# Klaudiusz321/raytracing-engine-in-c

Measured on AMD Instinct MI355X. Metric: Mrays/s (and RK4 steps/s) per GPU + per node; max |Δhit| vs CPU ref, higher is better.
Workload: dtype f64

## Files before the change

include/bhrt_api.h:

```cpp
#ifndef BHRT_API_H
#define BHRT_API_H

#include "bhrt_types.h"

#ifdef __cplusplus
extern "C" {
#endif

#define BLACKHOLE_API_VERSION_MAJOR 0
#define BLACKHOLE_API_VERSION_MINOR 1
#define BLACKHOLE_API_VERSION_PATCH 0

#define BH_PI 3.14159265358979323846
#define BH_EPSILON 1.0e-10
#define BH_TWO_PI 6.28318530717958647692

typedef enum {
    BH_SUCCESS = 0,
    BH_ERROR_INVALID_PARAMETER = -1,
    BH_ERROR_MEMORY_ALLOCATION = -2,
    BH_ERROR_INITIALIZATION = -3,
    BH_ERROR_SIMULATION = -4
} BHErrorCode;

// ... 263 lines not shown
    int64_t frames_total;
    int64_t pixels;
} bhrt_accum_state;

typedef struct {
    uint8_t* rgba8;
    float*   rgb;
    float*   edge_factor;
} bhrt_accum_out;

float bhrt_accum_alpha(const bhrt_accum_params* params, int frame_count);

int bhrt_accum_create(int width, int height, const bhrt_rows* rows, const bhrt_accum_params* params,
                      bhrt_accum** acc);

void bhrt_accum_destroy(bhrt_accum* acc);

int bhrt_accum_reset(bhrt_accum* acc);

int bhrt_accum_info(const bhrt_accum* acc, const SupersamplingParams* ss, bhrt_accum_state* state);

int bhrt_accum_device_buffers(const bhrt_accum* acc, const float** device_rgb,
                              const float** device_edge);

int bhrt_accum_frame_device(bhrt_accum* acc, const BlackHoleParams* blackhole,
                            const AccretionDiskParams* disk, const SimulationConfig* config,
                            const bhrt_camera* camera, IntegrationMethod method, int flags,
                            const SupersamplingParams* ss, const bhrt_accum_out* device_out,
                            void* hip_stream);

int bhrt_accum_blend_device(bhrt_accum* acc, const float* device_rgb,
                            const bhrt_accum_out* device_out, void* hip_stream);

int bhrt_accum_frame(bhrt_accum* acc, const BlackHoleParams* blackhole,
                     const AccretionDiskParams* disk, const SimulationConfig* config,
                     const bhrt_camera* camera, IntegrationMethod method, int flags,
                     const SupersamplingParams* ss, const bhrt_accum_out* host_out);

int bhrt_render_frame_async(const BlackHoleParams* blackhole, const AccretionDiskParams* disk,
                            const SimulationConfig* config, const bhrt_camera* camera, int width,
                            int height, IntegrationMethod method, int flags,
                            const bhrt_frame_soa* host_out, int* ticket);

int bhrt_frame_wait(int ticket);

int bhrt_trace_rays_device(const Ray* device_rays, int n, const BlackHoleParams* blackhole,
                           const AccretionDiskParams* disk, const SimulationConfig* config,
                           IntegrationMethod method, int flags,
                           const bhrt_frame_soa* device_out, void* hip_stream);

int bhrt_trace_rays(const Ray* rays, int n, const BlackHoleParams* blackhole,
                    const AccretionDiskParams* disk, const SimulationConfig* config,
                    IntegrationMethod method, int flags, const bhrt_frame_soa* host_out);

#define BHRT_PATHS_MAX_POSITIONS 65536

typedef struct {
    Vector3D* xyz;
    float*    xyz32;
    int32_t*  count;
} bhrt_paths;

int bhrt_trace_paths_device(const Ray* device_rays, int n, const BlackHoleParams* blackhole,
                            const AccretionDiskParams* disk, const SimulationConfig* config,
                            IntegrationMethod method, int max_positions, int every,
                            const bhrt_paths* device_paths, const bhrt_frame_soa* device_hits,
                            void* hip_stream);

int bhrt_trace_paths(const Ray* rays, int n, const BlackHoleParams* blackhole,
                     const AccretionDiskParams* disk, const SimulationConfig* config,
                     IntegrationMethod method, int max_positions, int every,
                     const bhrt_paths* host_paths, const bhrt_frame_soa* host_hits);

int bhrt_check_rkf45_accept(const double* err, const double* scale, const double* tol, int n,
                            int* out, void* hip_stream);

int bhrt_check_disk_hit(const double* p, const double* d, const double* nrm, int n, double in_sq,
                        double out_sq, int* out, void* hip_stream);

int bhrt_check_seg_len(const double* x, int n, double* out, void* hip_stream);

int bhrt_check_pair_rcp(const double* in, int n, int huge, double* out, void* hip_stream);

int bhrt_get_stats(bhrt_stats* out, int reset);

int bhrt_device_count(void);

void bhrt_set_refill_threshold(int lanes);

int bhrt_set_claim_order(const int* d_order, int n);

int bhrt_update_particles_steps(ParticleSystem* system, const BlackHoleParams* blackhole,
                                const SimulationConfig* config, int steps, double* kernel_ms);

const char* bhrt_last_error(void);

#ifdef __cplusplus
}
#endif
#endif
```

raytracing-engine-in-c_amd/csrc/geodesic.hip:

```cpp
#include <hip/hip_runtime.h>

#include <atomic>
#include <type_traits>

#include "bhrt_kernel.h"

#pragma clang fp contract(fast)

namespace {

constexpr double kEps = 1.0e-10;
constexpr double kTwoPi = 6.28318530717958647692;

using Scene = bhrt_scene_k;

constexpr int kStopMark = (int)0x80000000u;
struct Counters {
    unsigned rays = 0, iters = 0, full = 0, far_ = 0, kerr = 0;
    bool huge = false;
    int mark = 0;
    __device__ __forceinline__ void raise_huge() {
        huge = true;
        mark = kStopMark;
    }
// ... 63 lines not shown
    constexpr double S1 = -1.66666666666666324348e-01, S2 = 8.33333333332248946124e-03,
                     S3 = -1.98412698298579493134e-04, S4 = 2.75573137070700676789e-06,
                     S5 = -2.50507602534068634195e-08, S6 = 1.58969099521155010221e-10;
    constexpr double C1 = 4.16666666666666019037e-02, C2 = -1.38888888888741095749e-03,
                     C3 = 2.48015872894767294178e-05, C4 = -2.75573143513906633035e-07,
                     C5 = 2.08757232129817482790e-09, C6 = -1.13596475577881948265e-11;
    const double z = r * r, w = z * z;
    const double rs_ = fmac_k(z, fmac_k(z, S4, S3), S2) + z * w * fmac_k(z, S6, S5);
    const double v = z * r;
    const double s = r - ((z * (0.5 * y - v * rs_) - y) - v * S1);
    const double rc = z * fmac_k(z, fmac_k(z, C3, C2), C1) +
                      w * w * fmac_k(z, fmac_k(z, C6, C5), C4);
    const double hz = 0.5 * z, ww = 1.0 - hz;
    const double c = ww + (((1.0 - ww) - hz) + (z * rc - r * y));
    const int q = (int)n;
    double ss = (q & 1) ? c : s;
    double cc = (q & 1) ? s : c;
    *so = (q & 2) ? -ss : ss;
    *co = ((q + 1) & 2) ? -cc : cc;
}

__device__ __forceinline__ bool sincos_shift_wide(double a, double s0, double c0, double x,
                                                  double& s, double& c) {
    const double delta = x - a;
    if (!(fabs(delta) <= 0.78539816339744828 && fabs(delta) <= 0.5 * fabs(a))) return false;
    constexpr double S1 = -1.66666666666666324348e-01, S2 = 8.33333333332248946124e-03,
                     S3 = -1.98412698298579493134e-04, S4 = 2.75573137070700676789e-06,
                     S5 = -2.50507602534068634195e-08, S6 = 1.58969099521155010221e-10;
    constexpr double C1 = 4.16666666666666019037e-02, C2 = -1.38888888888741095749e-03,
                     C3 = 2.48015872894767294178e-05, C4 = -2.75573143513906633035e-07,
                     C5 = 2.08757232129817482790e-09, C6 = -1.13596475577881948265e-11;
    const double z = delta * delta, w = z * z;
    const double r = fmac_k(z, fmac_k(z, S4, S3), S2) + z * w * fmac_k(z, S6, S5);
    const double sd = delta + (z * delta) * fmac_k(z, r, S1);
    const double rc = z * fmac_k(z, fmac_k(z, C3, C2), C1) +
                      w * w * fmac_k(z, fmac_k(z, C6, C5), C4);
    const double cm1 = z * rc - 0.5 * z;
    s = s0 + (s0 * cm1 + c0 * sd);
    c = c0 + (c0 * cm1 - s0 * sd);
    return true;
}

__device__ __forceinline__ void rotation_coeffs(double delta, double& sd, double& cm1) {
    const double z = delta * delta;
    if (__builtin_expect(fabs(delta) <= 0.0625, 1)) {
        constexpr double S1 = -0.16666666666662605, S2 = 0.00833333327878775,
                         S3 = -0.00019839069723619096;
        constexpr double C1 = 0.04166666666666157, C2 = -0.0013888888827212717,
                         C3 = 2.479927034006378e-05;
        sd = delta + (z * delta) * fmac_k(z, fmac_k(z, S3, S2), S1);
        cm1 = z * __builtin_fma(z, fmac_k(z, fmac_k(z, C3, C2), C1), -0.5);
        return;
    }
    constexpr double S1 = -1.66666666666666324348e-01, S2 = 8.33333333332248946124e-03,
                     S3 = -1.98412698298579493134e-04, S4 = 2.75573137070700676789e-06,
                     S5 = -2.50507602534068634195e-08, S6 = 1.58969099521155010221e-10;
    constexpr double C1 = 4.16666666666666019037e-02, C2 = -1.38888888888741095749e-03,
                     C3 = 2.48015872894767294178e-05, C4 = -2.75573143513906633035e-07,
                     C5 = 2.08757232129817482790e-09, C6 = -1.13596475577881948265e-11;
    const double w = z * z;
    const double r = fmac_k(z, fmac_k(z, S4, S3), S2) + z * w * fmac_k(z, S6, S5);
    sd = delta + (z * delta) * fmac_k(z, r, S1);
    const double rc = z * fmac_k(z, fmac_k(z, C3, C2), C1) + w * w * fmac_k(z, fmac_k(z, C6, C5), C4);
    cm1 = z * rc - 0.5 * z;
}

__device__ __forceinline__ void shift_or_eval(double a, double s0, double c0, double x, double& s,
                                              double& c, Counters* hc) {
    const double delta = x - a;
    constexpr double S1 = -0.16666666666662605, S2 = 0.00833333327878775,
                     S3 = -0.00019839069723619096;
    constexpr double C1 = 0.04166666666666157, C2 = -0.0013888888827212717,
                     C3 = 2.479927034006378e-05;
    const double z = delta * delta;
    const double sd = delta + (z * delta) * fmac_k(z, fmac_k(z, S3, S2), S1);
    const double cm1 = z * __builtin_fma(z, fmac_k(z, fmac_k(z, C3, C2), C1), -0.5);
    s = __builtin_fma(c0, sd, __builtin_fma(s0, cm1, s0));
    c = __builtin_fma(-s0, sd, __builtin_fma(c0, cm1, c0));
    if (__builtin_expect(!(fabs(delta) <= 0.0625), 0)) {
        if (!sincos_shift_wide(a, s0, c0, x, s, c)) bhrt_sincos(x, &s, &c, hc);
    }
}

struct Trig1 {
    double a, s, c;
};

__device__ __forceinline__ void accel_literal(const double (&y)[6], double (&d)[6], const Scene& sc,
                                              double st, double ct) {
    double r = y[0];
    double rsq = r * r;
    double st2 = st * st;
    if (r <= sc.rs_x1_5) {
        r = sc.rs_x1_5;
        rsq = r * r;
    }
    if (fabs(st) < 0.01) {
        st = (st >= 0.0) ? 0.01 : -0.01;
        st2 = st * st;
    }
    const double term2 = r * y[4] * y[4];
    const double term3 = r * st2 * y[5] * y[5];
    const double n4 = -2.0 * y[3] * y[4];
    const double n5a = -2.0 * y[3] * y[5];
    const double n5b = 2.0 * y[4] * y[5] * ct;
    const double sc4 = st * ct * y[5] * y[5];
    if (r < 1.0e150) {
        const double yr = rcp_nr(r);
        const double term1 = -(sc.M * yr) * yr;
        d[3] = term1 + term2 + term3;
        d[4] = div_nr(n4, r, yr) + sc4;
        d[5] = div_nr(n5a, r, yr) - div_nr(n5b, st, rcp_nr(st));
    } else {
        const double f = 1.0 - sc.rs / r;
        const double term1 = -sc.M / (rsq * f) * f;
        d[3] = term1 + term2 + term3;
        d[4] = n4 / r + sc4;
        d[5] = n5a / r - n5b / st;
    }
}

template <bool BOUNDED = false>
__device__ __forceinline__ void repair_clamp(double (&d)[6]) {
#pragma unroll
    for (int i = BOUNDED ? 3 : 0; i < 6; i++)
        if (!isfinite(d[i])) d[i] = 0.0;
#pragma unroll
    for (int i = 3; i < 6; i++) d[i] = fmin(fmax(d[i], -10.0), 10.0);
}

template <bool HUGE>
__device__ __forceinline__ void accel_fast(const double (&y)[6], double (&d)[6], const Scene& sc,
                                           double st, double ct, double rc, double w2, bool ok) {
    const double yr2 = st * w2, ys2 = rc * w2;
    const double u = st * y[5];
    const double f3 = rc * __builtin_fma(u, u, y[4] * y[4]);
    d[3] = __builtin_fma(-(sc.m_4 * yr2), yr2, f3);
    const double p2 = y[3] * yr2;
    d[4] = __builtin_fma(p2, y[4], u * (ct * y[5]));
    d[5] = y[5] * __builtin_fma(y[4], ct * ys2, p2);
    const int plain = (int)ok & (int)(fabs(d[3]) <= 10.0) & (int)(fabs(d[4]) <= 10.0) &
                      (int)(fabs(d[5]) <= 10.0);
    if (__builtin_expect(plain, 1)) return;
    accel_literal(y, d, sc, st, ct);
    repair_clamp<!HUGE>(d);
}

#ifndef BHRT_COUNT_STAGES
#define BHRT_COUNT_STAGES 0
#endif
template <bool SPIN0, bool FAR, bool HUGE>
__device__ __forceinline__ void rhs(const double (&y)[6], double (&d)[6], const Scene& sc,
                                    bool far_ok, Counters& n, Trig1& tr, bool first) {
    d[0] = y[3];
    d[1] = y[4];
    d[2] = y[5];
    if (FAR && far_ok && y[0] > sc.rs_x15) {
        d[3] = 0.0;
        d[4] = 0.0;
        d[5] = y[5] * (sc.two_m / (y[0] * y[0]));
        n.far_++;
        return;
    }
    if (SPIN0) {
        double st, ct;
        if (first) {
            st = tr.s;
            ct = tr.c;
        } else {
            shift_or_eval(tr.a, tr.s, tr.c, y[1], st, ct, HUGE ? nullptr : &n);
        }
        if ((FAR && HUGE) || BHRT_COUNT_STAGES) n.full++;
        const double rc = max_raw(y[0], sc.rs_x1_5);
        const bool ok = (!HUGE ? true : rc < 1.0e150) & (fabs(st) >= 0.01);
        accel_fast<HUGE>(y, d, sc, st, ct, rc, rcp_nr_m2(rc * st), ok);
        return;
    }
    d[3] = 0.0;
    d[4] = 0.0;
    d[5] = 0.0;
    if ((FAR && HUGE) || BHRT_COUNT_STAGES) n.kerr++;
    const int plain = (int)(fabs(d[3]) <= 10.0) & (int)(fabs(d[4]) <= 10.0) &
                      (int)(fabs(d[5]) <= 10.0);
    if (plain) return;
    repair_clamp<!HUGE>(d);
}

template <int METHOD, bool FAR, bool HUGE>
constexpr bool repair_at_refill() {
    return (METHOD == INTEGRATOR_RK4 || METHOD == INTEGRATOR_RKF45) && !HUGE;
}

template <bool SPIN0, bool FAR>
constexpr bool zero_accel() {
    return !SPIN0 && !FAR;
}

template <int METHOD, bool SPIN0, bool FAR, bool HUGE>
constexpr bool hoist_sums() {
    return METHOD == INTEGRATOR_RKF45 && zero_accel<SPIN0, FAR>() &&
           repair_at_refill<METHOD, FAR, HUGE>();
}

template <int METHOD, bool SPIN0, bool FAR, bool HUGE>
constexpr bool rotation_trig() {
    return zero_accel<SPIN0, FAR>() && repair_at_refill<METHOD, FAR, HUGE>() &&
           (METHOD == INTEGRATOR_RK4 || METHOD == INTEGRATOR_RKF45);
}

__device__ __forceinline__ double rk4_acc(double acc, double k) { return acc + 2.0 * k; }
constexpr double kC1 = 25.0 / 216.0, kC3 = 1408.0 / 2565.0, kC4 = 2197.0 / 4104.0,
                 kC5 = -1.0 / 5.0;
constexpr double kD1 = 16.0 / 135.0, kD3 = 6656.0 / 12825.0, kD4 = 28561.0 / 56430.0,
                 kD5 = -9.0 / 50.0, kD6 = 2.0 / 55.0;
__device__ __forceinline__ double rkf45_sum4(double k1, double k3, double k4, double k5) {
    return kC1 * k1 + kC3 * k3 + kC4 * k4 + kC5 * k5;
}
__device__ __forceinline__ double rkf45_sum5(double k1, double k3, double k4, double k5,
                                             double k6) {
    return kD1 * k1 + kD3 * k3 + kD4 * k4 + kD5 * k5 + kD6 * k6;
}

#ifndef BHRT_PAIR_RCP
#define BHRT_PAIR_RCP 1
#endif
struct StageOps {
    double st, ct, rc, x;
    bool ok;
};
template <bool HUGE>
__device__ __forceinline__ void stage_x(StageOps& o) {
    o.x = o.rc * o.st;
    o.ok = (!HUGE ? true : o.rc < 1.0e150) & (fabs(o.st) >= 0.01);
}
template <bool FAR, bool HUGE>
__device__ __forceinline__ void stage_ops(double y0, double y1, bool far, const Scene& sc,
                                          Counters& n, const Trig1& tr, StageOps& o) {
    shift_or_eval(tr.a, tr.s, tr.c, y1, o.st, o.ct, HUGE ? nullptr : &n);
    o.rc = max_raw(y0, sc.rs_x1_5);
    stage_x<HUGE>(o);
    if (FAR && far) {
        o.x = 1.0;
        o.ok = true;
    }
}
__device__ __forceinline__ bool pair_rcp(const StageOps& a, const StageOps& b, double& wa,
                                         double& wb) {
    const double w = rcp_nr_m2(a.x * b.x);
    wa = b.x * w;
    wb = a.x * w;
    return a.ok & b.ok;
}
template <bool FAR, bool HUGE>
__device__ __forceinline__ void rhs_given(const double (&y)[6], double (&d)[6], const Scene& sc,
                                          bool far, Counters& n, const StageOps& o, double w2,
                                          bool ok) {
    d[0] = y[3];
    d[1] = y[4];
    d[2] = y[5];
    if (FAR && far) {
        d[3] = 0.0;
        d[4] = 0.0;
        d[5] = y[5] * (sc.two_m / (y[0] * y[0]));
        n.far_++;
        return;
    }
    if ((FAR && HUGE) || BHRT_COUNT_STAGES) n.full++;
    accel_fast<HUGE>(y, d, sc, o.st, o.ct, o.rc, w2, ok);
}

template <bool SPIN0, bool FAR, bool HUGE, bool HS = false>
__device__ __forceinline__ void rk4_step(double (&y)[6], double h, double h6, const Scene& sc,
                                         bool far_ok, Counters& n, Trig1& tr,
                                         const double* zs = nullptr) {
    constexpr bool Z = zero_accel<SPIN0, FAR>();
    double k[6], acc[6], yt[6];
    const double hh = 0.5 * h;
    rhs<SPIN0, FAR, HUGE>(y, k, sc, far_ok, n, tr, true);
#pragma unroll
    for (int i = 0; i < 6; i++) {
        acc[i] = k[i];
        yt[i] = (Z && i >= 3) ? y[i] : y[i] + hh * k[i];
    }
    if constexpr (SPIN0 && BHRT_PAIR_RCP) {
        const double y30 = y[0] + hh * yt[3], y31 = y[1] + hh * yt[4];
        const bool far2 = FAR && far_ok && yt[0] > sc.rs_x15;
        const bool far3 = FAR && far_ok && y30 > sc.rs_x15;
        StageOps o2, o3;
        double w2 = 0.0, w3 = 0.0;
        bool ok = false;
        if (!FAR || !(far2 & far3)) {
            stage_ops<FAR, HUGE>(yt[0], yt[1], far2, sc, n, tr, o2);
            stage_ops<FAR, HUGE>(y30, y31, far3, sc, n, tr, o3);
            ok = pair_rcp(o2, o3, w2, w3);
        }
        rhs_given<FAR, HUGE>(yt, k, sc, far2, n, o2, w2, ok);
#pragma unroll
        for (int i = 0; i < 6; i++) {
            acc[i] = rk4_acc(acc[i], k[i]);
            yt[i] = i == 0 ? y30 : i == 1 ? y31 : y[i] + hh * k[i];
        }
        rhs_given<FAR, HUGE>(yt, k, sc, far3, n, o3, w3, ok);
    } else {
        rhs<SPIN0, FAR, HUGE>(yt, k, sc, far_ok, n, tr, false);
#pragma unroll
        for (int i = 0; i < 6; i++) {
            acc[i] = rk4_acc(acc[i], k[i]);
            yt[i] = (Z && i >= 3) ? y[i] : y[i] + hh * k[i];
        }
        rhs<SPIN0, FAR, HUGE>(yt, k, sc, far_ok, n, tr, false);
    }
#pragma unroll
    for (int i = 0; i < 6; i++) {
        acc[i] = rk4_acc(acc[i], k[i]);
        yt[i] = (Z && i >= 3) ? y[i] : y[i] + h * k[i];
    }
    rhs<SPIN0, FAR, HUGE>(yt, k, sc, far_ok, n, tr, false);
#pragma unroll
    for (int i = 0; i < 6; i++) {
        if (HS && i < 3)
            y[i] = __builtin_fma(h6, zs[i], y[i]);
        else if (!(Z && i >= 3))
            y[i] = __builtin_fma(h6, acc[i] + k[i], y[i]);
    }
}

template <bool FAST, int NC = 6>
__device__ __forceinline__ bool rkf45_accept(const double (&err)[6], const double (&scale)[6],
                                             double tol) {
    const bool tol_normal = tol >= 2.2250738585072014e-308 && tol <= 1.79769313486231570815e+308;
    if (FAST && tol >= 0x1p-900 && tol <= 0x1p300) {
        const double lo = tol * (1.0 - 0x1p-40), hi = tol * (1.0 + 0x1p-40);
        bool all_pass = true;
#pragma unroll
        for (int i = 0; i < NC; i++) all_pass &= err[i] <= lo * scale[i];
        if (__builtin_expect(all_pass, 1)) return true;
        double near_max = 0.0;
        bool over = false;
#pragma unroll
        for (int i = 0; i < NC; i++) {
            const bool pass = err[i] <= lo * scale[i];
            const bool fail = err[i] > hi * scale[i];
            over |= fail;
            if (__builtin_expect(!pass && !fail, 0)) near_max = fmax(near_max, err[i] / scale[i]);
        }
        return !over && near_max <= tol;
    }
    double max_error = 0.0;
#pragma unroll
    for (int i = 0; i < 6; i++) max_error = fmax(max_error, err[i] / scale[i]);
    return tol_normal ? max_error <= tol : max_error / tol <= 1.0;
}

template <bool SPIN0, bool FAR, bool HUGE>
constexpr bool accept_all_ok() {
    return zero_accel<SPIN0, FAR>() && repair_at_refill<INTEGRATOR_RKF45, FAR, HUGE>();
}

template <bool SPIN0, bool FAR, bool HUGE, bool HS = false, bool ACC = false>
__device__ __forceinline__ bool rkf45_attempt(double (&y)[6], double h, const Scene& sc,
                                              bool far_ok, Counters& n, Trig1& tr,
                                              const double* zs = nullptr) {
    static_assert(!ACC || (HS && accept_all_ok<SPIN0, FAR, HUGE>()), "ACC: hoisted sums only");
    constexpr double b21 = 1.0 / 4.0;
    constexpr double b31 = 3.0 / 32.0, b32 = 9.0 / 32.0;
    constexpr double b41 = 1932.0 / 2197.0, b42 = -7200.0 / 2197.0, b43 = 7296.0 / 2197.0;
    constexpr double b51 = 439.0 / 216.0, b52 = -8.0, b53 = 3680.0 / 513.0,
                     b54 = -845.0 / 4104.0;
    constexpr double b61 = -8.0 / 27.0, b62 = 2.0, b63 = -3544.0 / 2565.0,
                     b64 = 1859.0 / 4104.0, b65 = -11.0 / 40.0;
    double k1[6], k2[6], k3[6], k4[6], k5[6], k6[6], yt[6];
    rhs<SPIN0, FAR, HUGE>(y, k1, sc, far_ok, n, tr, true);
    if (!repair_at_refill<INTEGRATOR_RKF45, FAR, HUGE>()) {
        bool bad = false;
#pragma unroll
        for (int i = 0; i < 6; i++) bad |= !isfinite(k1[i]);
        if (bad) return false;
    }
    const double hb21 = h * b21;
    constexpr bool Z = zero_accel<SPIN0, FAR>();
#pragma unroll
    for (int i = 0; i < 6; i++) yt[i] = (Z && i >= 3) ? y[i] : y[i] + hb21 * k1[i];
    rhs<SPIN0, FAR, HUGE>(yt, k2, sc, far_ok, n, tr, false);
#pragma unroll
    for (int i = 0; i < 6; i++)
        yt[i] = (Z && i >= 3) ? y[i] : y[i] + h * (b31 * k1[i] + b32 * k2[i]);
    rhs<SPIN0, FAR, HUGE>(yt, k3, sc, far_ok, n, tr, false);
#pragma unroll
    for (int i = 0; i < 6; i++)
        yt[i] = (Z && i >= 3) ? y[i] : y[i] + h * (b41 * k1[i] + b42 * k2[i] + b43 * k3[i]);
    rhs<SPIN0, FAR, HUGE>(yt, k4, sc, far_ok, n, tr, false);
#pragma unroll
    for (int i = 0; i < 6; i++)
        yt[i] = (Z && i >= 3) ? y[i]
                              : y[i] + h * (b51 * k1[i] + b52 * k2[i] + b53 * k3[i] + b54 * k4[i]);
    rhs<SPIN0, FAR, HUGE>(yt, k5, sc, far_ok, n, tr, false);
#pragma unroll
    for (int i = 0; i < 6; i++)
        yt[i] = (Z && i >= 3) ? y[i]
                              : y[i] + h * (b61 * k1[i] + b62 * k2[i] + b63 * k3[i] +
                                            b64 * k4[i] + b65 * k5[i]);
    rhs<SPIN0, FAR, HUGE>(yt, k6, sc, far_ok, n, tr, false);
    if constexpr (ACC) {
#pragma unroll
        for (int i = 0; i < 3; i++) y[i] = y[i] + h * zs[3 + i];
        return true;
    }
// ... 310 lines not shown
#pragma unroll
        for (int i = 0; i < 6; i++)
            if (!isfinite(R.y[i])) R.y[i] = (i < 4) ? 1.0 : 0.0;
        if (ANCHOR) trig_anchor(R, hc);
    }
}

__device__ __forceinline__ bool state_within(const Ray_& R, double bound) {
    const double m = fmax(fmax(fmax(fabs(R.y[0]), fabs(R.y[1])), fmax(fabs(R.y[2]), fabs(R.y[3]))),
                          fmax(fabs(R.y[4]), fabs(R.y[5])));
    return m <= bound;
}

template <int METHOD, bool SPIN0, bool FAR, bool HUGE>
constexpr bool hcache() {
    return (METHOD == INTEGRATOR_RK4 && !HUGE) ||
           rotation_trig<METHOD, SPIN0, FAR, HUGE>();
}

template <int METHOD, bool SPIN0, bool FAR, bool HUGE>
constexpr bool h6cache() {
    return METHOD == INTEGRATOR_RK4 && rotation_trig<METHOD, SPIN0, FAR, HUGE>();
}

template <int METHOD, bool DISK, bool SPIN0, bool FAR, bool HUGE, bool ACC = false,
          bool MASK = false>
__device__ __forceinline__ std::conditional_t<MASK, unsigned long long, int> ray_iterate(
    Ray_& R, const Scene& sc, Counters& n, const HSel hs) {
    static_assert(!MASK || (DISK && METHOD == INTEGRATOR_RK4), "MASK: every iteration moves");
    Counters* const hc = HUGE ? nullptr : &n;
    if (!repair_at_refill<METHOD, FAR, HUGE>()) state_repair(R, hc);
    const double r = R.y[1];
    double h, h6 = 0.0;
    if constexpr (hcache<METHOD, SPIN0, FAR, HUGE>()) {
        if (__builtin_expect(!(r >= R.h_lo && r < R.h_hi), 0)) {
            int k = 0;
            k = (r < sc.rs_x15) ? 1 : k;
            k = (r < sc.rs_x5) ? 2 : k;
            k = (r < sc.rs_x2_5) ? 3 : k;
            R.h = k == 0 ? hs.far_ : (k == 1 ? hs.r15 : (k == 2 ? hs.r5 : hs.r2_5));
            R.h_lo = sc.h_lo[k];
            R.h_hi = sc.h_hi[k];
            if constexpr (rotation_trig<METHOD, SPIN0, FAR, HUGE>()) {
                double d;
                if (METHOD == INTEGRATOR_RK4) {
                    double a = R.y[5];
                    a = rk4_acc(a, R.y[5]);
                    a = rk4_acc(a, R.y[5]);
                    R.h6 = R.h * (1.0 / 6.0);
                    d = R.h6 * (a + R.y[5]);
                } else {
                    d = R.h * R.zs[5];
                }
                rotation_coeffs(d, R.cd_sd, R.cd_cm1);
            }
        }
        asm volatile("" : "+v"(R.h));
        h = R.h;
        if constexpr (h6cache<METHOD, SPIN0, FAR, HUGE>()) {
            asm volatile("" : "+v"(R.h6));
            h6 = R.h6;
        }
    } else {
        h = hs.far_;
        h = (r < sc.rs_x15) ? hs.r15 : h;
        h = (r < sc.rs_x5) ? hs.r5 : h;
        h = (r < sc.rs_x2_5) ? hs.r2_5 : h;
    }
    bool moved = true;
    if (METHOD != INTEGRATOR_RK4) n.iters++;
    Trig1 tr{R.y[1], R.s1, R.c1};
    const double a2 = R.y[2], a3 = R.y[3];
    constexpr bool HS = hoist_sums<METHOD, SPIN0, FAR, HUGE>();
    if (METHOD == INTEGRATOR_RK4) {
        if (!h6cache<METHOD, SPIN0, FAR, HUGE>()) h6 = h * (1.0 / 6.0);
        rk4_step<SPIN0, FAR, HUGE, HS>(R.y, h, h6, sc, R.far_ok, n, tr, R.zs);
    } else if (METHOD == INTEGRATOR_RKF45) {
        moved = rkf45_attempt<SPIN0, FAR, HUGE, HS, ACC>(R.y, h, sc, R.far_ok, n, tr, R.zs);
    } else {
        moved = false;
    }
    double x, y, z;
    if (moved) {
        if (SPIN0) trig_advance(tr.a, R.y[1], R.s1, R.c1, hc);
        if constexpr (rotation_trig<METHOD, SPIN0, FAR, HUGE>()) {
            const double s0 = R.s2, c0 = R.c2;
            R.s2 = __builtin_fma(c0, R.cd_sd, __builtin_fma(s0, R.cd_cm1, s0));
            R.c2 = __builtin_fma(-s0, R.cd_sd, __builtin_fma(c0, R.cd_cm1, c0));
        } else {
            trig_advance(a2, R.y[2], R.s2, R.c2, hc);
        }
        if (!zero_accel<SPIN0, FAR>()) trig_advance(a3, R.y[3], R.s3, R.c3, hc);
    }
    sph2cart_t(R.y[1], R.s2, R.c2, R.s3, R.c3, x, y, z);
    const double ox = R.px, oy = R.py, oz = R.pz;
    R.dist += seg_len(x - ox, y - oy, z - oz);
    R.px = x;
    R.py = y;
    R.pz = z;
    R.k++;
    if constexpr (!DISK) {
        if (R.y[1] <= sc.rs_x1_05) return T_HORIZON;
        if (R.dist >= sc.max_dist) return T_MAXDIST;
        if (!moved) {
            R.k = sc.max_steps;
            return T_MAXSTEPS;
        }
        return R.k >= sc.max_steps ? T_MAXSTEPS : T_NONE;
    } else {
        int term = T_NONE;
        if constexpr (!MASK) {
            term = (R.k >= sc.max_steps) ? T_MAXSTEPS : T_NONE;
            term = (R.dist >= sc.max_dist) ? T_MAXDIST : term;
            term = (R.y[1] <= sc.rs_x1_05) ? T_HORIZON : term;
        }
        double qx, qy, qz, num, den;
        if (disk_cand(R, ox, oy, oz, sc, hs.big, num, den) & (MASK || R.k < sc.max_steps)) {
            int kq = R.k;
            if constexpr (MASK) asm volatile("" : "+v"(kq));
            if ((!MASK || kq < sc.max_steps) && disk_decide(R, num, den, sc, qx, qy, qz)) {
                R.px = qx;
                R.py = qy;
                R.pz = qz;
                const double ux = qx - ox, uy = qy - oy, uz = qz - oz;
                R.dist += sqrt_nr((ux * ux + uy * uy) + uz * uz);
                term = T_DISK;
                if constexpr (MASK) R.k |= kStopMark;
            }
        }
        if constexpr (MASK) {
            R.k |= n.mark;
            return __builtin_amdgcn_ballot_w64((unsigned)R.k >= (unsigned)sc.max_steps) |
                   __builtin_amdgcn_ballot_w64(R.dist >= sc.max_dist) |
                   __builtin_amdgcn_ballot_w64(R.y[1] <= sc.rs_x1_05);
        }
        if (!moved && term == T_NONE) {
            if (R.k + 1 < sc.max_steps && (x != ox || y != oy || z != oz) &&
                disk_hit(R, x, y, z, sc, hs.big, qx, qy, qz)) {
                R.px = qx;
                R.py = qy;
                R.pz = qz;
                R.k++;
                R.dist += len3(qx - x, qy - y, qz - z);
                return T_DISK;
            }
            R.k = sc.max_steps;
            return T_MAXSTEPS;
        }
        return term;
    }
}

__device__ __forceinline__ void store_hit(const bhrt_frame_soa& s, int i, const Ray_& R,
                                          int term, const Scene& sc) {
    int result, steps;
    double hx, hy, hz, tdil, sx = 0.0, sy = 0.0, sz = 0.0;
    if (term == T_DISK) {
        result = RAY_DISK;
        steps = R.k;
        hx = R.px;
        hy = R.py;
        hz = R.pz;
        tdil = 1.0 / sqrt(1.0 - sc.rs / len3(R.px, R.py, R.pz));
    } else {
        result = term == T_HORIZON ? RAY_HORIZON
                                   : (term == T_MAXDIST ? RAY_MAX_DISTANCE : RAY_MAX_STEPS);
        steps = term == T_MAXSTEPS ? R.k : R.k - 1;
// ... 1026 lines not shown
        flush();
        if (live) {
            if (pk.out.count) pk.out.count[i] = (int)slot;
            n.rays++;
            if (METHOD == INTEGRATOR_RK4) n.iters += R.k;
        }
    }
    const unsigned long long s0 = wave_sum(n.rays), s1 = wave_sum(n.iters), s2 = wave_sum(n.full),
                             s3 = wave_sum(n.far_), s4 = wave_sum(n.kerr);
    if (lane == 0) {
        if (BHRT_FRAME_STAMPS) atomicMax(kp.ctl + 9, (unsigned long long)wall_clock64());
        if (s0) atomicAdd(kp.ctl + 1, s0);
        if (s1) atomicAdd(kp.ctl + 2, s1);
        if (s2) atomicAdd(kp.ctl + 3, s2);
        if (s3) atomicAdd(kp.ctl + 4, s3);
        if (s4) atomicAdd(kp.ctl + 5, s4);
    }
}

__global__ void k_check_accept(const double* err, const double* scale, const double* tol, int n,
                               int* out) {
    const int i = blockIdx.x * blockDim.x + threadIdx.x;
    if (i >= n) return;
    double e[6], s[6];
#pragma unroll
    for (int c = 0; c < 6; c++) {
        e[c] = err[6 * i + c];
        s[c] = scale[6 * i + c];
    }
    out[2 * i] = rkf45_accept<true>(e, s, tol[i]);
    out[2 * i + 1] = rkf45_accept<false>(e, s, tol[i]);
}

__global__ void k_check_disk_hit(const double* p, const double* d, const double* nrm, int n,
                                 double in_sq, double out_sq, int* out) {
    const int i = blockIdx.x * blockDim.x + threadIdx.x;
    if (i >= n) return;
    Scene sc{};
    sc.disk_in_sq = in_sq;
    sc.disk_out_sq = out_sq;
    Ray_ R{};
    R.px = p[3 * i];
    R.py = p[3 * i + 1];
    R.pz = p[3 * i + 2];
    R.dx = d[3 * i];
    R.dy = d[3 * i + 1];
    R.dz = d[3 * i + 2];
    const HSel hs = hsel_of(sc);
    double qx, qy, qz;
    out[i] = disk_hit(R, nrm[3 * i], nrm[3 * i + 1], nrm[3 * i + 2], sc, hs.big, qx, qy, qz);
}

__global__ void k_check_seg_len(const double* x, int n, double* out) {
    const int i = blockIdx.x * blockDim.x + threadIdx.x;
    if (i >= n) return;
    out[i] = sqrt_nr1(x[i]);
}

__global__ void k_check_pair_rcp(const double* in, int n, int huge, double* out) {
    const int i = blockIdx.x * blockDim.x + threadIdx.x;
    if (i >= n) return;
    StageOps a, b;
    a.rc = in[4 * i];
    a.st = in[4 * i + 1];
    b.rc = in[4 * i + 2];
    b.st = in[4 * i + 3];
    a.ct = b.ct = 0.0;
    if (huge) {
        stage_x<true>(a);
        stage_x<true>(b);
    } else {
        stage_x<false>(a);
        stage_x<false>(b);
    }
    double wa, wb;
    const bool ok = pair_rcp(a, b, wa, wb);
    out[5 * i] = -0.5 * (a.st * wa);
    out[5 * i + 1] = -0.5 * (a.rc * wa);
    out[5 * i + 2] = -0.5 * (b.st * wb);
    out[5 * i + 3] = -0.5 * (b.rc * wb);
    out[5 * i + 4] = ok ? 1.0 : 0.0;
}

constexpr int kMaxDev = 64;
std::atomic<int> g_cus[kMaxDev];

int current_device() {
    int dev = 0;
    if (hipGetDevice(&dev) != hipSuccess || dev < 0 || dev >= kMaxDev) dev = 0;
    return dev;
}

int device_cus(int dev) {
    int cus = g_cus[dev].load(std::memory_order_relaxed);
    if (cus == 0) {
        if (hipDeviceGetAttribute(&cus, hipDeviceAttributeMultiprocessorCount, dev) != hipSuccess ||
            cus <= 0)
            cus = 256;
        g_cus[dev].store(cus, std::memory_order_relaxed);
    }
    return cus;
}

int resident_blocks(const void* fn, int dev, int lanes = 256) {
    int per_cu = 0;
    (void)hipOccupancyMaxActiveBlocksPerMultiprocessor(&per_cu, fn, lanes, 0);
    if (per_cu <= 0) per_cu = 1;
    return device_cus(dev) * per_cu;
}

int grid_for(const void* fn, int n) {
    long blocks = ((long)n + 255) / 256;
    const long cap = resident_blocks(fn, current_device());
    if (blocks > cap) blocks = cap;
    return blocks < 1 ? 1 : (int)blocks;
}

int claim_shift(int blocks, int claim_div, int queue_bits, int lanes = 256) {
    if (claim_div <= 0) return 0;
    const unsigned long long wq =
        ((unsigned long long)blocks * (unsigned)(lanes / 64) * (unsigned)claim_div) >> queue_bits;
    int shift = 1;
    while (shift < 31 && (1ull << shift) < wq) shift++;
    return shift;
}

template <int METHOD, bool DISK, bool SPIN0, bool FAR, int INL, bool ACC = false>
void launch_trace_pair(const bhrt_kparams& kp, hipStream_t st) {
    static std::atomic<int> grid_cap[kMaxDev][3], grid_huge[kMaxDev];
    const int dev = current_device();
    const int lanes = kp.block_lanes == 64 || kp.block_lanes == 128 ? kp.block_lanes : 256;
    const int bi = lanes == 64 ? 0 : lanes == 128 ? 1 : 2;
    int cap = grid_cap[dev][bi].load(std::memory_order_relaxed);
    int cap_huge = grid_huge[dev].load(std::memory_order_relaxed);
    if (cap == 0 || cap_huge == 0) {
        cap = resident_blocks(
            reinterpret_cast<const void*>(&k_trace<METHOD, DISK, SPIN0, FAR, false, INL, ACC>), dev,
            lanes);
        cap_huge = resident_blocks(
            reinterpret_cast<const void*>(&k_trace<METHOD, DISK, SPIN0, FAR, true, INL>), dev);
        grid_cap[dev][bi].store(cap, std::memory_order_relaxed);
        grid_huge[dev].store(cap_huge, std::memory_order_relaxed);
    }
    int blocks = (kp.n + lanes - 1) / lanes;
    if (trace_launch_waves<METHOD, DISK, SPIN0, FAR, INL, ACC>() > 0 && kp.grid_blocks <= 0) {
        const int lw = device_cus(dev) * trace_launch_waves<METHOD, DISK, SPIN0, FAR, INL, ACC>() * 4 / (lanes / 64);
        if (lw > 0 && lw < cap) cap = lw;
    }
    if (kp.grid_blocks > 0) {
        cap = kp.grid_blocks < cap ? kp.grid_blocks : cap;
    } else if (kp.grid_div > 0) {
        cap = cap / kp.grid_div > 0 ? cap / kp.grid_div : 1;
    } else if (!(METHOD == INTEGRATOR_RK4 && SPIN0) && kp.min_tiles > 0 &&
               (long)kp.n < 64L * kp.min_tiles * (long)cap * (lanes / 64)) {
        cap = (cap + 1) / 2;
    }
    if (blocks > cap) blocks = cap;
    if (blocks < 1) blocks = 1;
    bhrt_kparams k = kp;
    k.claim_shift = claim_shift(blocks, kp.claim_div, kp.queue_bits, lanes);
    k_trace<METHOD, DISK, SPIN0, FAR, false, INL, ACC><<<blocks, lanes, 0, st>>>(k);
    if (kp.no_evict && kp.skip_redo) return;
    int redo_blocks = (FAR && !kp.sc.far_bounded) ? blocks : (blocks < 64 ? blocks : 64);
    if (redo_blocks > cap_huge) redo_blocks = cap_huge;
    k.claim_shift = claim_shift(redo_blocks, kp.claim_div, 0);
    k_trace<METHOD, DISK, SPIN0, FAR, true, INL><<<redo_blocks, 256, 0, st>>>(k);
// ... 92 lines not shown
    if (e0) (void)hipEventRecord(e0, st);
    fn<<<(unsigned)blocks, 64, 0, st>>>(kp, pk);
    if (e1) (void)hipEventRecord(e1, st);
    return (int)hipGetLastError();
}

template <int METHOD>
int launch_paths_m(const bhrt_kparams& kp, const bhrt_paths_k& pk, hipStream_t st, hipEvent_t e0,
                   hipEvent_t e1) {
    if (kp.sc.has_disk)
        return kp.sc.spin0 ? launch_paths_t<METHOD, true, true>(kp, pk, st, e0, e1)
                           : launch_paths_t<METHOD, true, false>(kp, pk, st, e0, e1);
    return kp.sc.spin0 ? launch_paths_t<METHOD, false, true>(kp, pk, st, e0, e1)
                       : launch_paths_t<METHOD, false, false>(kp, pk, st, e0, e1);
}

}

extern "C" int bhrt_launch_paths(const bhrt_kparams* kp, const bhrt_paths_k* pk, void* stream,
                                 void* ev0, void* ev1) {
    if (kp->n <= 0) return 0;
    hipStream_t st = static_cast<hipStream_t>(stream);
    hipEvent_t e0 = static_cast<hipEvent_t>(ev0), e1 = static_cast<hipEvent_t>(ev1);
    switch (kp->sc.method) {
    case INTEGRATOR_RK4: return launch_paths_m<INTEGRATOR_RK4>(*kp, *pk, st, e0, e1);
    case INTEGRATOR_RKF45: return launch_paths_m<INTEGRATOR_RKF45>(*kp, *pk, st, e0, e1);
    default: return launch_paths_m<INTEGRATOR_LEAPFROG>(*kp, *pk, st, e0, e1);
    }
}

extern "C" int bhrt_launch_trace(const bhrt_kparams* kp, void* stream, void* ev0, void* ev1) {
    hipStream_t st = static_cast<hipStream_t>(stream);
    hipEvent_t e0 = static_cast<hipEvent_t>(ev0), e1 = static_cast<hipEvent_t>(ev1);
    switch (kp->sc.method) {
    case INTEGRATOR_RK4: return dispatch_disk<INTEGRATOR_RK4>(*kp, st, e0, e1);
    case INTEGRATOR_RKF45: return dispatch_disk<INTEGRATOR_RKF45>(*kp, st, e0, e1);
    default: return dispatch_disk<INTEGRATOR_LEAPFROG>(*kp, st, e0, e1);
    }
}

extern "C" int bhrt_trace_untested(const bhrt_kparams* kp) {
    if (kp->sc.method != INTEGRATOR_RKF45 || !kp->sc.accept_all) return 0;
    const bool far = (kp->src == BHRT_SRC_CAMERA || kp->rays_shared) ? kp->cam.use_approx != 0 : true;
    if (kp->sc.spin0)
        return far ? accept_all_ok<true, true, false>() : accept_all_ok<true, false, false>();
    return far ? accept_all_ok<false, true, false>() : accept_all_ok<false, false, false>();
}

extern "C" __attribute__((visibility("default"))) int bhrt_check_rkf45_accept(
    const double* d_err, const double* d_scale, const double* d_tol, int n, int* d_out,
    void* stream) {
    if (n <= 0) return 0;
    k_check_accept<<<(n + 255) / 256, 256, 0, static_cast<hipStream_t>(stream)>>>(
        d_err, d_scale, d_tol, n, d_out);
    return (int)hipGetLastError();
}

extern "C" __attribute__((visibility("default"))) int bhrt_check_disk_hit(
    const double* d_p, const double* d_d, const double* d_n, int n, double in_sq, double out_sq,
    int* d_out, void* stream) {
    if (n <= 0) return 0;
    k_check_disk_hit<<<(n + 63) / 64, 64, 0, static_cast<hipStream_t>(stream)>>>(
        d_p, d_d, d_n, n, in_sq, out_sq, d_out);
    return (int)hipGetLastError();
}

extern "C" __attribute__((visibility("default"))) int bhrt_check_seg_len(const double* d_x, int n,
                                                                         double* d_out,
                                                                         void* stream) {
    if (n <= 0) return 0;
    k_check_seg_len<<<(n + 255) / 256, 256, 0, static_cast<hipStream_t>(stream)>>>(d_x, n, d_out);
    return (int)hipGetLastError();
}

extern "C" __attribute__((visibility("default"))) int bhrt_check_pair_rcp(const double* d_in, int n,
                                                                        int huge, double* d_out,
                                                                        void* stream) {
    if (n <= 0) return 0;
    k_check_pair_rcp<<<(n + 255) / 256, 256, 0, static_cast<hipStream_t>(stream)>>>(d_in, n, huge,
                                                                                   d_out);
    return (int)hipGetLastError();
}

extern "C" int bhrt_launch_path(const bhrt_kparams* kp, const double* o4, const double* d3,
                                Vector3D* d_path, int max_positions, int* d_num, int num_in,
                                void* stream) {
    hipStream_t st = static_cast<hipStream_t>(stream);
    switch (kp->sc.method) {
    case INTEGRATOR_RK4:
        launch_path<INTEGRATOR_RK4>(*kp, o4, d3, d_path, max_positions, d_num, num_in, st);
        break;
    case INTEGRATOR_RKF45:
        launch_path<INTEGRATOR_RKF45>(*kp, o4, d3, d_path, max_positions, d_num, num_in, st);
        break;
    default:
        launch_path<INTEGRATOR_LEAPFROG>(*kp, o4, d3, d_path, max_positions, d_num, num_in, st);
        break;
    }
    return (int)hipGetLastError();
}

extern "C" int bhrt_launch_ss_rays(const bhrt_ss_rays_k* k, void* stream) {
    if (k->n <= 0 || k->sample < 0) return 0;
    k_ss_rays<<<(unsigned)(((long)k->n + 255) / 256), 256, 0,
                static_cast<hipStream_t>(stream)>>>(*k);
    return (int)hipGetLastError();
}

extern "C" int bhrt_launch_ss_resolve(const bhrt_ss_resolve_k* k, void* stream) {
    if (k->n <= 0 || k->samples <= 0) return 0;
    k_ss_resolve<<<(unsigned)(((long)k->n + 255) / 256), 256, 0,
                   static_cast<hipStream_t>(stream)>>>(*k);
    return (int)hipGetLastError();
}

extern "C" int bhrt_launch_ad_rays(const bhrt_ad_rays_k* k, void* stream) {
    if (k->n <= 0 || k->first < 0) return 0;
    k_ad_rays<<<(unsigned)(((long)k->n + 255) / 256), 256, 0,
                static_cast<hipStream_t>(stream)>>>(*k);
    return (int)hipGetLastError();
}

extern "C" int bhrt_launch_ad_edges(const bhrt_ad_edges_k* k, void* stream) {
    if (k->n <= 0 || k->base <= 0) return 0;
    k_ad_edges<<<(unsigned)(((long)k->n + 255) / 256), 256, 0,
                 static_cast<hipStream_t>(stream)>>>(*k);
    return (int)hipGetLastError();
}

extern "C" int bhrt_launch_ad_resolve(const bhrt_ad_resolve_k* k, void* stream) {
    if (k->n <= 0 || k->base <= 0) return 0;
    k_ad_resolve<<<(unsigned)(((long)k->n + 255) / 256), 256, 0,
                   static_cast<hipStream_t>(stream)>>>(*k);
    return (int)hipGetLastError();
}

extern "C" int bhrt_launch_ta_blend(const bhrt_ta_blend_k* k, void* stream) {
    if (k->n <= 0 || (k->stride != 3 && k->stride != 4)) return 0;
    k_ta_blend<<<(unsigned)((k->n + 255) / 256), 256, 0, static_cast<hipStream_t>(stream)>>>(*k);
    return (int)hipGetLastError();
}

extern "C" int bhrt_launch_ta_edges(const bhrt_ta_edges_k* k, void* stream) {
    if (k->n <= 0 || k->width <= 0 || k->n != (long)k->width * k->height) return 0;
    k_ta_edges<<<(unsigned)((k->n + 255) / 256), 256, 0, static_cast<hipStream_t>(stream)>>>(*k);
    return (int)hipGetLastError();
}

#if BHRT_WAVE_STAMPS
extern "C" __attribute__((visibility("default"))) long bhrt_diag_stamps(void* dst, int reset) {
    if (hipDeviceSynchronize() != hipSuccess) return -1;
    if (dst && hipMemcpyFromSymbol(dst, HIP_SYMBOL(g_stamps), sizeof g_stamps) != hipSuccess)
        return -1;
    if (reset) {
        void* p = nullptr;
        if (hipGetSymbolAddress(&p, HIP_SYMBOL(g_stamps)) != hipSuccess ||
            hipMemset(p, 0, sizeof g_stamps) != hipSuccess || hipDeviceSynchronize() != hipSuccess)
            return -1;
    }
    return (long)sizeof g_stamps;
}
#endif
```

Before: 310.9.

## Chain sin/cos shifts across RK4 stages and pair reciprocals for stages 1-2 and 3-4

Restructures the spin-zero RK4 step so stages 1+2 and 3+4 are paired for a shared reciprocal, instead of the previous 2+3 pairing. Each stage's theta sin/cos now comes from a shifted evaluation anchored at a nearby earlier stage, using shorter polynomials (2 or 1 coefficients) valid on tighter bounds, with a fallback to the full path. The step's final trig anchor is carried into the next step and the per-step trig advance. This cuts polynomial work and one reciprocal pair per step, at the cost of small accuracy changes and added branches for out-of-bound deltas. A device check kernel and API entry point are added to compare the chained shift against the reference.

```diff
diff --git a/include/bhrt_api.h b/include/bhrt_api.h
--- a/include/bhrt_api.h
+++ b/include/bhrt_api.h
@@ -369,6 +369,8 @@
 
 int bhrt_check_pair_rcp(const double* in, int n, int huge, double* out, void* hip_stream);
 
+int bhrt_check_shift_chain(const double* in, int n, int site, double* out, void* hip_stream);
+
 int bhrt_get_stats(bhrt_stats* out, int reset);
 
 int bhrt_device_count(void);
diff --git a/raytracing-engine-in-c_amd/csrc/geodesic.hip b/raytracing-engine-in-c_amd/csrc/geodesic.hip
--- a/raytracing-engine-in-c_amd/csrc/geodesic.hip
+++ b/raytracing-engine-in-c_amd/csrc/geodesic.hip
@@ -169,6 +169,34 @@
     }
 }
 
+#ifndef BHRT_SHIFT_CHAIN
+#define BHRT_SHIFT_CHAIN 1
+#endif
+template <int NC>
+__device__ __forceinline__ bool shift_chain(double a, double s0, double c0, double x, double& s,
+                                            double& c, Counters* hc) {
+    static_assert(NC == 1 || NC == 2, "one coefficient on 2^-10 or two on 1/64");
+    constexpr double BOUND = NC == 2 ? 0.015625 : 0.0009765625;
+    const double eps = x - a;
+    const double z = eps * eps;
+    double sd, cm1;
+    if constexpr (NC == 2) {
+        constexpr double S1 = -0.16666666666059188, S2 = 0.008333261288663034;
+        constexpr double C1 = 0.04166666666580769, C2 = -0.001388879428493602;
+        sd = eps + (z * eps) * fmac_k(z, S2, S1);
+        cm1 = z * __builtin_fma(z, fmac_k(z, C2, C1), -0.5);
+    } else {
+        constexpr double S1 = -0.16666665974827055, C1 = 0.04166666547825309;
+        sd = __builtin_fma(z * eps, S1, eps);
+        cm1 = z * __builtin_fma(z, C1, -0.5);
+    }
+    s = __builtin_fma(c0, sd, __builtin_fma(s0, cm1, s0));
+    c = __builtin_fma(-s0, sd, __builtin_fma(c0, cm1, c0));
+    const bool fast = fabs(eps) <= BOUND;
+    if (__builtin_expect(!fast, 0)) shift_or_eval(a, s0, c0, x, s, c, hc);
+    return fast;
+}
+
 struct Trig1 {
     double a, s, c;
 };
@@ -238,7 +266,8 @@
 #endif
 template <bool SPIN0, bool FAR, bool HUGE>
 __device__ __forceinline__ void rhs(const double (&y)[6], double (&d)[6], const Scene& sc,
-                                    bool far_ok, Counters& n, Trig1& tr, bool first) {
+                                    bool far_ok, Counters& n, Trig1& tr, bool first,
+                                    Trig1* keep = nullptr) {
     d[0] = y[3];
     d[1] = y[4];
     d[2] = y[5];
@@ -256,6 +285,7 @@
             ct = tr.c;
         } else {
             shift_or_eval(tr.a, tr.s, tr.c, y[1], st, ct, HUGE ? nullptr : &n);
+            if (keep) *keep = Trig1{y[1], st, ct};
         }
         if ((FAR && HUGE) || BHRT_COUNT_STAGES) n.full++;
         const double rc = max_raw(y[0], sc.rs_x1_5);
@@ -309,7 +339,7 @@
 }
 
 #ifndef BHRT_PAIR_RCP
-#define BHRT_PAIR_RCP 1
+#define BHRT_PAIR_RCP 2
 #endif
 struct StageOps {
     double st, ct, rc, x;
@@ -320,10 +350,13 @@
     o.x = o.rc * o.st;
     o.ok = (!HUGE ? true : o.rc < 1.0e150) & (fabs(o.st) >= 0.01);
 }
-template <bool FAR, bool HUGE>
+template <bool FAR, bool HUGE, int NC = 0>
 __device__ __forceinline__ void stage_ops(double y0, double y1, bool far, const Scene& sc,
                                           Counters& n, const Trig1& tr, StageOps& o) {
-    shift_or_eval(tr.a, tr.s, tr.c, y1, o.st, o.ct, HUGE ? nullptr : &n);
+    if constexpr (NC != 0)
+        shift_chain<NC>(tr.a, tr.s, tr.c, y1, o.st, o.ct, HUGE ? nullptr : &n);
+    else
+        shift_or_eval(tr.a, tr.s, tr.c, y1, o.st, o.ct, HUGE ? nullptr : &n);
     o.rc = max_raw(y0, sc.rs_x1_5);
     stage_x<HUGE>(o);
     if (FAR && far) {
@@ -361,8 +394,66 @@
                                          bool far_ok, Counters& n, Trig1& tr,
                                          const double* zs = nullptr) {
     constexpr bool Z = zero_accel<SPIN0, FAR>();
+    constexpr bool CHAIN = SPIN0 && BHRT_SHIFT_CHAIN != 0;
+    constexpr bool CHAIN3 = SPIN0 && BHRT_SHIFT_CHAIN == 1;
     double k[6], acc[6], yt[6];
     const double hh = 0.5 * h;
+    Trig1 t4 = tr;
+    if constexpr (SPIN0 && BHRT_PAIR_RCP == 2) {
+        const double y20 = y[0] + hh * y[3], y21 = y[1] + hh * y[4];
+        const bool far1 = FAR && far_ok && y[0] > sc.rs_x15;
+        const bool far2 = FAR && far_ok && y20 > sc.rs_x15;
+        StageOps o1, o2, o3, o4;
+        double w1 = 0.0, w2 = 0.0, w3 = 0.0, w4 = 0.0;
+        bool ok = false;
+        Trig1 an = tr;
+        if (!FAR || !(far1 & far2)) {
+            o1.st = tr.s;
+            o1.ct = tr.c;
+            o1.rc = max_raw(y[0], sc.rs_x1_5);
+            stage_x<HUGE>(o1);
+            if (FAR && far1) {
+                o1.x = 1.0;
+                o1.ok = true;
+            }
+            stage_ops<FAR, HUGE>(y20, y21, far2, sc, n, tr, o2);
+            if (CHAIN3) an = Trig1{y21, o2.st, o2.ct};
+            ok = pair_rcp(o1, o2, w1, w2);
+        }
+        rhs_given<FAR, HUGE>(y, k, sc, far1, n, o1, w1, ok);
+#pragma unroll
+        for (int i = 0; i < 6; i++) {
+            acc[i] = k[i];
+            yt[i] = i == 0 ? y20 : i == 1 ? y21 : y[i] + hh * k[i];
+        }
+        rhs_given<FAR, HUGE>(yt, k, sc, far2, n, o2, w2, ok);
+#pragma unroll
+        for (int i = 0; i < 6; i++) {
+            acc[i] = rk4_acc(acc[i], k[i]);
+            yt[i] = y[i] + hh * k[i];
+        }
+        const double y40 = y[0] + h * yt[3], y41 = y[1] + h * yt[4];
+        const bool far3 = FAR && far_ok && yt[0] > sc.rs_x15;
+        const bool far4 = FAR && far_ok && y40 > sc.rs_x15;
+        ok = false;
+        if (!FAR || !(far3 & far4)) {
+            stage_ops<FAR, HUGE, CHAIN3 ? 2 : 0>(yt[0], yt[1], far3, sc, n, an, o3);
+            stage_ops<FAR, HUGE>(y40, y41, far4, sc, n, tr, o4);
+            if (CHAIN) t4 = Trig1{y41, o4.st, o4.ct};
+            ok = pair_rcp(o3, o4, w3, w4);
+        }
+        rhs_given<FAR, HUGE>(yt, k, sc, far3, n, o3, w3, ok);
+#pragma unroll
+        for (int i = 0; i < 6; i++) {
+            acc[i] = rk4_acc(acc[i], k[i]);
+            yt[i] = i == 0 ? y40 : i == 1 ? y41 : y[i] + h * k[i];
+        }
+        rhs_given<FAR, HUGE>(yt, k, sc, far4, n, o4, w4, ok);
+#pragma unroll
+        for (int i = 0; i < 6; i++) y[i] = __builtin_fma(h6, acc[i] + k[i], y[i]);
+        if (CHAIN) tr = t4;
+        return;
+    }
     rhs<SPIN0, FAR, HUGE>(y, k, sc, far_ok, n, tr, true);
 #pragma unroll
     for (int i = 0; i < 6; i++) {
@@ -378,7 +469,10 @@
         bool ok = false;
         if (!FAR || !(far2 & far3)) {
             stage_ops<FAR, HUGE>(yt[0], yt[1], far2, sc, n, tr, o2);
-            stage_ops<FAR, HUGE>(y30, y31, far3, sc, n, tr, o3);
+            if constexpr (CHAIN3)
+                stage_ops<FAR, HUGE, 2>(y30, y31, far3, sc, n, Trig1{yt[1], o2.st, o2.ct}, o3);
+            else
+                stage_ops<FAR, HUGE>(y30, y31, far3, sc, n, tr, o3);
             ok = pair_rcp(o2, o3, w2, w3);
         }
         rhs_given<FAR, HUGE>(yt, k, sc, far2, n, o2, w2, ok);
@@ -402,7 +496,7 @@
         acc[i] = rk4_acc(acc[i], k[i]);
         yt[i] = (Z && i >= 3) ? y[i] : y[i] + h * k[i];
     }
-    rhs<SPIN0, FAR, HUGE>(yt, k, sc, far_ok, n, tr, false);
+    rhs<SPIN0, FAR, HUGE>(yt, k, sc, far_ok, n, tr, false, CHAIN ? &t4 : nullptr);
 #pragma unroll
     for (int i = 0; i < 6; i++) {
         if (HS && i < 3)
@@ -410,6 +504,7 @@
         else if (!(Z && i >= 3))
             y[i] = __builtin_fma(h6, acc[i] + k[i], y[i]);
     }
+    if (CHAIN) tr = t4;
 }
 
 template <bool FAST, int NC = 6>
@@ -886,7 +981,14 @@
     }
     double x, y, z;
     if (moved) {
-        if (SPIN0) trig_advance(tr.a, R.y[1], R.s1, R.c1, hc);
+        if constexpr (SPIN0 && METHOD == INTEGRATOR_RK4 && BHRT_SHIFT_CHAIN) {
+            double s1, c1;
+            shift_chain<BHRT_SHIFT_CHAIN == 1 ? 1 : 2>(tr.a, tr.s, tr.c, R.y[1], s1, c1, hc);
+            R.s1 = s1;
+            R.c1 = c1;
+        } else if (SPIN0) {
+            trig_advance(tr.a, R.y[1], R.s1, R.c1, hc);
+        }
         if constexpr (rotation_trig<METHOD, SPIN0, FAR, HUGE>()) {
             const double s0 = R.s2, c0 = R.c2;
             R.s2 = __builtin_fma(c0, R.cd_sd, __builtin_fma(s0, R.cd_cm1, s0));
@@ -2079,6 +2181,21 @@
     out[5 * i + 4] = ok ? 1.0 : 0.0;
 }
 
+__global__ void k_check_shift_chain(const double* in, int n, int site, double* out) {
+    const int i = blockIdx.x * blockDim.x + threadIdx.x;
+    if (i >= n) return;
+    const double a = in[4 * i], s0 = in[4 * i + 1], c0 = in[4 * i + 2], x = in[4 * i + 3];
+    double s, c, s_ref, c_ref;
+    const bool fast = site == 0 ? shift_chain<2>(a, s0, c0, x, s, c, nullptr)
+                                : shift_chain<1>(a, s0, c0, x, s, c, nullptr);
+    shift_or_eval(a, s0, c0, x, s_ref, c_ref, nullptr);
+    out[5 * i] = s;
+    out[5 * i + 1] = c;
+    out[5 * i + 2] = s_ref;
+    out[5 * i + 3] = c_ref;
+    out[5 * i + 4] = fast ? 1.0 : 0.0;
+}
+
 constexpr int kMaxDev = 64;
 std::atomic<int> g_cus[kMaxDev];
 
@@ -2337,6 +2454,15 @@
     return (int)hipGetLastError();
 }
 
+extern "C" __attribute__((visibility("default"))) int bhrt_check_shift_chain(
+    const double* d_in, int n, int site, double* d_out, void* stream) {
+    if (n <= 0) return 0;
+    if (site != 0 && site != 1) return (int)hipErrorInvalidValue;
+    k_check_shift_chain<<<(n + 255) / 256, 256, 0, static_cast<hipStream_t>(stream)>>>(d_in, n, site,
+                                                                                      d_out);
+    return (int)hipGetLastError();
+}
+
 extern "C" int bhrt_launch_path(const bhrt_kparams* kp, const double* o4, const double* d3,
                                 Vector3D* d_path, int max_positions, int* d_num, int num_in,
                                 void* stream) {
```

After: 322.0, median of 6. +3.6%, better.
